# bruAristimunha/Synthetic-Sleep-EEG-Signal-Generation-using-Latent-Diffusion-Models

Measured on AMD Instinct MI355X. Metric: EEG windows/sec (LDM train step), higher is better.
Workload: dtype bf16; 1 GPU; LDM train step on raw (B,1,3072) windows: frozen AutoencoderKL[32,32,64] encode+sample x scale, add_noise, config_ldm.yaml UNet (30.5M params, latent_channels=1) fwd+bwd, epsilon MSE, Adam lr 1e-4 [BASELINE configs[2]/[3]: per-GPU batch 256 = global 2048 / 8]; per_gpu_batch=256, global_batch=256, latent_len=768, parallelism=dp1

## Files before the change

include/eegldm.h:

```cpp
#ifndef EEGLDM_H
#define EEGLDM_H
#include <stdint.h>
#ifdef __cplusplus
extern "C" {
#endif

#define EEGLDM_ABI_VERSION 8

enum { EEGLDM_F32 = 0, EEGLDM_BF16 = 1, EEGLDM_F16 = 2 };
enum {
  EEGLDM_OK = 0,
  EEGLDM_ERR_INVALID = -1,
  EEGLDM_ERR_HIP = -2,
  EEGLDM_ERR_UNSUPPORTED = -3,
  EEGLDM_ERR_NOMEM = -4
};
enum { EEGLDM_PRED_EPSILON = 0, EEGLDM_PRED_V = 1, EEGLDM_PRED_SAMPLE = 2 };

typedef struct eegldm_ctx eegldm_ctx;
typedef struct eegldm_unet eegldm_unet;
typedef struct eegldm_aekl eegldm_aekl;
typedef struct eegldm_disc eegldm_disc;
typedef struct eegldm_block eegldm_block;

int eegldm_abi_version(void);
const char* eegldm_last_error(void);
int eegldm_ctx_create(int hip_device, void* hip_stream, int own_stream, eegldm_ctx** out);
void* eegldm_ctx_stream(const eegldm_ctx*);
int eegldm_ctx_destroy(eegldm_ctx* ctx);
int eegldm_ctx_sync(eegldm_ctx* ctx);
int eegldm_timer_start(eegldm_ctx* ctx);
int eegldm_timer_stop_ms(eegldm_ctx* ctx, float* ms_host);
int eegldm_prof_enable(eegldm_ctx* ctx, int on);
int eegldm_prof_summary(eegldm_ctx* ctx, int kernel_class, double* flops_host, double* ms_host, int* launches_host);
int eegldm_prof_bracket_overhead_ms(eegldm_ctx* ctx, double* ms_host);
int eegldm_prof_dump(eegldm_ctx* ctx, const char* path_host);
int eegldm_debug_reload_env(void);
int eegldm_debug_gn_last_route(int backward, int* out6_host);
int eegldm_debug_bn_last_route(int backward, int* out8_host);
int eegldm_debug_dconv_last_route(int which, int* out8_host);
int eegldm_debug_aekl_last_route(const eegldm_aekl*, int* out10_host);
int eegldm_debug_aekl_encode_route(const eegldm_aekl*, int* out3_host);
int eegldm_debug_pre_conv3(eegldm_ctx*, int dtype, const void* x, const double* in_stats, const float* gamma, const float* beta, const void* w,
                           const float* bias, const void* resid, void* y, double* out_stats, int B, int L, int Cin, int Cout, float eps);
int eegldm_debug_sample_stats(eegldm_ctx*, int dtype, const void* x, long n_per_sample, int B, double* stats);
int eegldm_debug_bn_stats_from_parts(eegldm_ctx*, const float* parts_dev, int nb, float* stats, float* running_mean, float* running_var,
                                     float* num_batches_tracked, long rows, int C);
int eegldm_debug_disc_tail_fwd(eegldm_ctx*, int dtype, const void* y, long ldy, const float* gamma, const float* beta, const float* stats,
                               const float* w3, const float* bias, float slope, float* logits, int B, int L, int C);
int eegldm_debug_disc_tail_bwd(eegldm_ctx*, int dtype, const void* y, long ldy, const float* gamma, const float* beta, const float* stats,
                               const float* w3, float slope, const float* dlogits, void* dy, long lddy, float* dgamma, float* dbeta,
                               float* dw3, float* dbias, int B, int L, int C);
int eegldm_debug_disc_head_bwd(eegldm_ctx*, int dtype, const void* da, long ldda, const void* x, const void* w, const float* bias, float slope,
                               float* dw, float* db, float* dx, int B, int L, int Lo, int C0, int stride);
int eegldm_debug_conv1d_fwd_colstats(eegldm_ctx*, const void* x, long ldx, const void* w, const float* bias, void* y, long ldy,
                                     int B, int Lin, int Cin, int Cout, int K, int stride, int pad_l, int pad_r,
                                     const float* rowvec, long ld_rowvec, const void* resid, long ld_resid, int dtype,
                                     float* col_parts_dev, int* col_nparts_host);

int eegldm_ncl_to_nlc(eegldm_ctx*, const float* src_ncl, void* dst_nlc, long ld_dst, int B, int C, int L, int dst_dtype);
int eegldm_nlc_to_ncl(eegldm_ctx*, const void* src_nlc, long ld_src, float* dst_ncl, int B, int C, int L, int src_dtype);
int eegldm_pack_conv_weight(eegldm_ctx*, const float* w_ref, float* w_packed, int Cout, int Cin, int K);
int eegldm_unpack_conv_weight(eegldm_ctx*, const float* w_packed, float* w_ref, int Cout, int Cin, int K);
int eegldm_cast(eegldm_ctx*, const float* src, void* dst, long n, int dst_dtype);

int eegldm_conv1d_pack_kblocked(eegldm_ctx*, const void* w, void* w_kblocked, int Cout, int Cin, int dtype);
int eegldm_conv1d_pack_kblocked_k(eegldm_ctx*, const void* w, void* w_kblocked, int Cout, int Cin, int K, int dtype);
int eegldm_conv1d_forget_kblocked(eegldm_ctx*, const void* w);
int eegldm_conv1d_pack_stride2(eegldm_ctx*, const void* w, void* w_fwd, void* w_dgrad, int Cout, int Cin, int dtype);
int eegldm_conv1d_pack_dgrad(eegldm_ctx*, const void* w, void* w_dgrad, int Cout, int Cin, int dtype);
int eegldm_conv1d_pack_dgrad_k(eegldm_ctx*, const void* w, void* w_dgrad, int Cout, int Cin, int K, int dtype);
// ... 386 lines not shown
```

synthetic-sleep-eeg-signal-generation-using-latent-diffusion-models_amd/_lib.py:

```python
import ctypes as C
import os

_HERE = os.path.dirname(os.path.abspath(__file__))
LIB_PATH = os.environ.get("EEGLDM_LIB") or os.path.join(_HERE, "libeegldm.so")

F32, BF16, F16 = 0, 1, 2
PRED = {"epsilon": 0, "v_prediction": 1, "sample": 2}


class LibraryMissing(RuntimeError):
    pass


def _load():
    import torch
    if not os.path.exists(LIB_PATH):
        raise LibraryMissing(f"{LIB_PATH} not found: build it with `make` (python -c 'import __graft_entry__ as g; g.build()')")
    return C.CDLL(LIB_PATH)


lib = _load()
lib.eegldm_last_error.restype = C.c_char_p
if hasattr(lib, "eegldm_ctx_stream"):
    lib.eegldm_ctx_stream.restype = C.c_void_p
if hasattr(lib, 'eegldm_unet_num_params'):
    lib.eegldm_unet_num_params.restype = C.c_long

_vp, _i, _l, _f = C.c_void_p, C.c_int, C.c_long, C.c_float
SIGNATURES = {
    "eegldm_abi_version": [],
    "eegldm_last_error": [],
    "eegldm_ctx_create": [_i, _vp, _i, C.POINTER(_vp)],
    "eegldm_ctx_stream": [_vp],
    "eegldm_ctx_destroy": [_vp],
    "eegldm_ctx_sync": [_vp],
    "eegldm_timer_start": [_vp],
    "eegldm_timer_stop_ms": [_vp, C.POINTER(_f)],
    "eegldm_prof_enable": [_vp, _i],
    "eegldm_prof_summary": [_vp, _i, C.POINTER(C.c_double), C.POINTER(C.c_double), C.POINTER(_i)],
    "eegldm_prof_bracket_overhead_ms": [_vp, C.POINTER(C.c_double)],
    "eegldm_prof_dump": [_vp, C.c_char_p],
    "eegldm_debug_reload_env": [],
    "eegldm_debug_gn_last_route": [_i, _vp],
    "eegldm_debug_bn_last_route": [_i, _vp],
    "eegldm_debug_dconv_last_route": [_i, _vp],
    "eegldm_debug_aekl_last_route": [_vp, _vp],
    "eegldm_debug_aekl_encode_route": [_vp, _vp],
    "eegldm_debug_pre_conv3": [_vp, _i, _vp, _vp, _vp, _vp, _vp, _vp, _vp, _vp, _vp, _i, _i, _i, _i, _f],
    "eegldm_debug_sample_stats": [_vp, _i, _vp, _l, _i, _vp],
    "eegldm_debug_bn_stats_from_parts": [_vp, _vp, _i, _vp, _vp, _vp, _vp, _l, _i],
    "eegldm_debug_disc_tail_fwd": [_vp, _i, _vp, _l, _vp, _vp, _vp, _vp, _vp, _f, _vp, _i, _i, _i],
    "eegldm_debug_disc_tail_bwd": [_vp, _i, _vp, _l, _vp, _vp, _vp, _vp, _f, _vp, _vp, _l, _vp, _vp, _vp, _vp, _i, _i, _i],
    "eegldm_debug_disc_head_bwd": [_vp, _i, _vp, _l, _vp, _vp, _vp, _f, _vp, _vp, _vp, _i, _i, _i, _i, _i],
    "eegldm_debug_conv1d_fwd_colstats": [_vp, _vp, _l, _vp, _vp, _vp, _l, _i, _i, _i, _i, _i, _i, _i, _i, _vp, _l, _vp, _l, _i, _vp, _vp],
    "eegldm_ncl_to_nlc": [_vp, _vp, _vp, _l, _i, _i, _i, _i],
    "eegldm_nlc_to_ncl": [_vp, _vp, _l, _vp, _i, _i, _i, _i],
    "eegldm_pack_conv_weight": [_vp, _vp, _vp, _i, _i, _i],
    "eegldm_conv1d_pack_kblocked": [_vp, _vp, _vp, _i, _i, _i],
    "eegldm_conv1d_pack_kblocked_k": [_vp, _vp, _vp, _i, _i, _i, _i],
    "eegldm_batchnorm_lrelu_fwd": [_vp, _vp, _l, _vp, _vp, _vp, _vp, _vp, _vp, _vp, _l, _l, _i, _f, _i, _i],
    "eegldm_batchnorm_lrelu_bwd": [_vp, _vp, _l, _vp, _vp, _vp, _vp, _l, _vp, _l, _vp, _vp, _l, _i, _f, _i],
    "eegldm_kl_reparam_fwd": [_vp, _vp, _vp, _vp, _vp, _vp, _vp, _l, _i, _i],
    "eegldm_kl_reparam_bwd": [_vp, _vp, _vp, _vp, _vp, _vp, _vp, _vp, _l, _f, _i],
    "eegldm_avgpool2_fwd": [_vp, _vp, _l, _vp, _l, _i, _i, _i, _i],
    "eegldm_avgpool2_bwd": [_vp, _vp, _l, _vp, _l, _i, _i, _i, _i],
    "eegldm_nearest2_fwd": [_vp, _vp, _l, _vp, _l, _i, _i, _i, _i],
    "eegldm_nearest2_bwd": [_vp, _vp, _l, _vp, _l, _i, _i, _i, _i],
    "eegldm_conv1d_skip_fwd": [_vp, _vp, _l, _vp, _vp, _vp, _l, _vp, _vp, _vp, _l, _i, _i, _i, _i, _i, _vp, _l, _i],
    "eegldm_comm_unique_id": [_vp],
    "eegldm_comm_create": [_vp, _vp, _i, _i, _vp],
    "eegldm_comm_destroy": [_vp],
    "eegldm_comm_rank": [_vp],
    "eegldm_comm_world": [_vp],
    "eegldm_comm_allreduce_mean_f32": [_vp, _vp, _l, _l],
    "eegldm_comm_broadcast_f32": [_vp, _vp, _l, _i],
    "eegldm_comm_wait": [_vp],
# ... 313 lines not shown
```

synthetic-sleep-eeg-signal-generation-using-latent-diffusion-models_amd/csrc/internal.h:

```cpp
#pragma once
#include "common.h"

int ew_temb(eegldm_ctx*, const int64_t* t, void* out, int B, int dim, int dtype);
int ew_silu(eegldm_ctx*, const float* x, void* y, long n, int dtype);
int ew_silu_bwd(eegldm_ctx*, const float* dy, const float* x, void* dx, long n, int dtype);
int eeg_det_buffer(eegldm_ctx*, size_t bytes, float** out);
int ew_fold_partials_det(eegldm_ctx*, const float* parts, int nparts, long stride, int off, int n, float* total);
int ew_colsum(eegldm_ctx*, const void* x, long ldx, float* out_ps, long ldo, float* total, int B, int L, int C, int dtype);
int ew_softmax(eegldm_ctx*, const float* S, void* P, long rows, int n, int dtype);
int ew_softmax_bwd(eegldm_ctx*, const float* dP, const void* P, void* dS, long rows, int n, float alpha, int dtype);
int ew_add_rows(eegldm_ctx*, void* dst, long ldd, const void* src, long lds, long rows, int C, int dtype);
int ew_dropout_rows(eegldm_ctx*, void* x, long ld, long rows, int C, float p, uint64_t seed, uint64_t offset, int dtype);
int ew_film_silu_fwd(eegldm_ctx*, const void* hn, long ldh, const float* emb, long lde, void* a, long lda, int B, int L, int C, int dtype);
int ew_film_silu_bwd(eegldm_ctx*, const void* hn, long ldh, const float* emb, long lde, const void* da, long ldda, void* dhn, long lddh,
                     float* demb, long ldde, int B, int L, int C, int dtype);
int ew_copy_rows(eegldm_ctx*, void* dst, long ldd, const void* src, long lds, long rows, int C, int dtype);
int ew_ncl2_to_nlc(eegldm_ctx*, const float* x, int Cx, const float* context, int Cc, int rows, void* dst, long ld, int B, int L, int dtype);
int ew_label_emb_add(eegldm_ctx*, float* emb, long ld, const int64_t* y, const float* table, int B, int te, int K);
int ew_label_emb_grad(eegldm_ctx*, const float* demb, long ld, const int64_t* y, int B, int te, int K, float* dtable);
int ew_label_dropout(eegldm_ctx*, const int64_t* y, int64_t* out, int B, float p, int64_t null_class, uint64_t seed, uint64_t offset);
int ew_emb_gather(eegldm_ctx*, const float* table, const int64_t* y, int K, int w, float* out, int B);

bool conv_is_thin(int Cin, int Cout, int dtype);
struct KbDesc { long off; long chunk0; int cout, cin; };
int kblk_pack(eegldm_ctx* ctx, const void* w_plain, void* w_packed, const KbDesc* d_table, int n, long total_chunks);
int kblk_pack_one(eegldm_ctx* ctx, const void* w_plain, void* w_packed, int Cout, int Cin, int taps = 3);
int kblk_pack_t(eegldm_ctx* ctx, const void* w_plain, void* w_packed, const KbDesc* d_table, int n, long total_chunks);
int kblk_pack_t_one(eegldm_ctx* ctx, const void* w_plain, void* w_packed, int Cout, int Cin, int taps = 3);
int s2ws_pack(eegldm_ctx* ctx, const void* w, void* wf, void* wd, int Cout, int Cin);
int dconv_run(eegldm_ctx*, int dtype, bool dgrad, const void* in, long ldin, const void* w, const float* bias,
              const void* resid, long ldr, void* out, long ldout, int B, int Lin, int Lout, int Cin, int Cout, int K,
              int stride, int pad_l, float act_slope = 0.f);
bool dconv_fuses_act(int dtype, int Cin, int Cout, int K, long ldout);
int dconv_wgrad(eegldm_ctx*, int dtype, const void* x, long ldx, const void* dy, long lddy, float* dw, int B, int Lin,
                int Lout, int Cin, int Cout, int K, int stride, int pad_l, float* dbias, int* bias_done);
bool dconv_wgrad_tinyv_ok(int Cin, int Cout, int K);

struct SkinnyGn { const float2* part; const float* gamma; const float* beta; int cpg; float eps; int silu;
                  const float2* part_b = nullptr; int nqa = 0; };
struct SkinnyExt { const void* x2; long ldx2; const void* w2; int Cin2; const float* bias2; };
bool conv_skinny_takes(int dtype, int Cin, int Cout, int taps, int B, int L);
int conv_skinny_ex(eegldm_ctx* ctx, int dtype, const void* x, long ldx, const void* w, int Cin, int Cout, int taps, const float* bias,
                   const float* rowvec, long ld_rowvec, const void* resid, long ldr, void* y, long ldy, int B, int L,
                   const SkinnyGn* gn, float2* part_out, const SkinnyExt* ext = nullptr);
int conv_skinny_try(eegldm_ctx* ctx, int dtype, const void* x, long ldx, const void* w, int Cin, int Cout, int taps, const float* bias,
                    const float* rowvec, long ld_rowvec, const void* resid, long ldr, void* y, long ldy, int B, int L);
int conv_ws2_try(eegldm_ctx*, int dtype, int dgrad, const void* x, const void* w, const float* bias, void* y, int B, int Lo,
                 float* col_parts = nullptr, int* col_nparts = nullptr);
int conv_ws_try(eegldm_ctx*, int dtype, const void* x, long ldx, const void* w, int Cin, int Cout, int transposed, const float* bias,
                const float* rowvec, long ld_rowvec, const void* resid, long ldr, void* y, long ldy, int B, int L,
                float* col_parts = nullptr, int* col_nparts = nullptr);

int op_conv_fwd(eegldm_ctx*, int dtype, const void* x, long ldx, const void* w, const float* bias, void* y, long ldy,
                int B, int Lin, int Cin, int Cout, int K, int stride, int pad_l, int pad_r,
// ... 58 lines not shown
```

synthetic-sleep-eeg-signal-generation-using-latent-diffusion-models_amd/csrc/unet.hip:

```cpp
#include <string.h>

#include <string>
#include <vector>

#include "net.h"

namespace {
constexpr int GN_G = 32;
struct Layer { int kind; ResDesc r; AttnDesc a; RsDesc s; };
inline int layer_cin(const Layer& l) { return l.kind == 0 ? l.r.cin : (l.kind == 1 ? l.a.c : l.s.c); }
inline int layer_cout(const Layer& l) { return l.kind == 0 ? l.r.cout : (l.kind == 1 ? l.a.c : l.s.c); }
inline int layer_len(const Layer& l, int L) {
  if (l.kind == 0) return l.r.updown == 1 ? L / 2 : (l.r.updown == 2 ? L * 2 : L);
  if (l.kind == 2) return l.s.up ? L * 2 : L / 2;
  return L;
}
struct Block { std::vector<Layer> layers; int cin, cout; };
}

struct eegldm_unet : NetBase {
  eegldm_unet_cfg cfg;
  int mc, te;
  long off_emb_w = 0, off_emb_b = 0, off_te0_w, off_te0_b, off_te2_w, off_te2_b, off_cin_w, off_cin_b, off_out_gw, off_out_gb, off_out_w, off_out_b;
  std::vector<Block> in_blocks, out_blocks; Block mid;
// ... 233 lines not shown
extern "C" int eegldm_unet_destroy(eegldm_unet* u) {
  if (!u) return 0;
  sampler_release(u);
  if (u->fuse_stats) (void)hipFree(u->fuse_stats);
  delete u;
  return 0;
}
extern "C" int eegldm_unet_set_dropout(eegldm_unet* u, float p, uint64_t seed) {
  EEG_CHECK(u, "null unet");
  EEG_CHECK(p >= 0.f && p < 1.f, "dropout probability %g outside [0, 1)", (double)p);
  u->dropout = p; u->drop_seed = seed; u->drop_ctr = 0;
  return 0;
}
extern "C" int eegldm_unet_num_entries(const eegldm_unet* u) { return (int)u->entries.size(); }
extern "C" long eegldm_unet_num_params(const eegldm_unet* u) { return u->nparams; }
extern "C" int eegldm_unet_set_grad_hook(eegldm_unet* u, eegldm_grad_hook fn, void* user) {
  EEG_CHECK(u, "null unet");
  u->grad_hook = fn; u->grad_hook_user = user;
  return 0;
}
extern "C" int eegldm_unet_entry(const eegldm_unet* u, int i, char* name, int cap, long* offset, long* numel, int* ndim, int shape[3]) {
  return entry_query(u, i, name, cap, offset, numel, ndim, shape);
}
extern "C" int eegldm_unet_bind(eegldm_unet* u, float* params, float* grads) {
  EEG_CHECK(u && params, "null argument");
  sampler_release(u);
  return u->bind(params, grads);
}
extern "C" int eegldm_unet_sync_weights(eegldm_unet* u) {
  EEG_CHECK(u, "null argument");
  return u->sync_weights();
}

static int embed_chain(eegldm_unet* u, const int64_t* tsteps, const int64_t* labels, int n, float* e0, float* h1e, float* a1e, float* emb,
                       float* semb, float* emb_all) {
  eegldm_ctx* ctx = u->ctx; const int mc = u->mc, te = u->te, F = EEGLDM_F32;
  EEG_TRY(ew_temb(ctx, tsteps, e0, n, mc, F));
  EEG_TRY(op_linear(ctx, F, e0, mc, u->P(u->off_te0_w), mc, u->P(u->off_te0_b), h1e, te, n, te, mc, 1));
  EEG_TRY(ew_silu(ctx, h1e, a1e, (long)n * te, F));
  EEG_TRY(op_linear(ctx, F, a1e, te, u->P(u->off_te2_w), te, u->P(u->off_te2_b), emb, te, n, te, te, 1));
  if (u->num_classes > 0) EEG_TRY(ew_label_emb_add(ctx, emb, te, labels, u->P(u->off_label), n, te, u->num_classes));
  EEG_TRY(ew_silu(ctx, emb, semb, (long)n * te, F));
  return op_linear(ctx, F, semb, te, u->P(u->off_emb_w), te, u->P(u->off_emb_b), emb_all, u->etot, n, u->etot, te, 1);
}
int unet_emb_width(const eegldm_unet* u) { return u->etot; }
long unet_embed_work_floats(const eegldm_unet* u) { return (long)u->mc + 4L * u->te; }
int unet_embed_table(eegldm_unet* u, const int64_t* tsteps_dev, const int64_t* labels_dev, int n, float* table, float* work) {
  EEG_CHECK(u && u->params && tsteps_dev && table && work && n > 0, "bad argument");
  EEG_CHECK(u->num_classes == 0 || labels_dev, "a class-conditional UNet's embedding rows need labels");
  const long te = u->te;
  float* e0 = work; float* h1e = e0 + (long)n * u->mc; float* a1e = h1e + n * te; float* emb = a1e + n * te; float* semb = emb + n * te;
  return embed_chain(u, tsteps_dev, labels_dev, n, e0, h1e, a1e, emb, semb, table);
}
void unet_set_shared_emb(eegldm_unet* u, const float* rows, long ld) { u->emb_shared = rows; u->emb_shared_ld = ld; }

struct LabelArg { const int64_t* y = nullptr; float p_uncond = 0.f; int64_t null_class = 0; uint64_t seed = 0, offset = 0; };
static int unet_forward_impl(eegldm_unet* u, const float* x, const int64_t* tsteps, const LabelArg& lab, float* y, int B, int L, int training) {
  EEG_CHECK(u && x && tsteps && y, "null argument");
  EEG_CHECK(u->params, "bind parameters first");
  EEG_CHECK(B > 0 && L > 0 && (L % (1 << (u->cfg.n_mult - 1))) == 0, "L=%d must be divisible by 2^(levels-1)", L);
  EEG_CHECK(!u->context || B % u->context_rows == 0, "a forward of %d rows cannot share %d context rows (B %% rows != 0)", B, u->context_rows);
  eegldm_ctx* ctx = u->ctx; const int dt = u->dtype; const int mc = u->mc, te = u->te;
  u->arena.reset(); u->rt.clear(); u->at.clear(); u->st.clear(); u->in_out.clear(); u->cat.clear();
  u->B = B; u->L = L; u->have_tape = false; u->training = training != 0;

  {
    EEG_ENV_VAR(bool, no_fuse, getenv("EEGLDM_NO_EVAL_GN_FUSE") != nullptr);
    u->eval_fuse = !training && !no_fuse && (dt == EEGLDM_BF16 || dt == EEGLDM_F16); u->fused_used = false; u->fuse_used = 0; u->part_reg.clear();
    if (u->eval_fuse) {
// ... 63 lines not shown
    EEG_TRY(block_forward(u, u->out_blocks[j], u->cat[j], B, Lj, dst));
    h = dst;
  }
  u->h_last = h;
  ALLOC_OR_FAIL(u->st_out, (float*)u->arena.alloc(sizeof(float) * 2 * B * GN_G));
  ALLOC_OR_FAIL(u->a_out.p, u->alloc_act((long)B * L, mc)); u->a_out.ld = mc; u->a_out.C = mc;
  EEG_TRY(eegldm_groupnorm_fwd(ctx, h.p, h.ld, u->P(u->off_out_gw), u->P(u->off_out_gb), u->a_out.p, mc, u->st_out, B, L, mc, GN_G, GN_EPS, 1, 0, nullptr, 0, dt));
  Arena::Mark mk = u->arena.mark();
  void* yo; ALLOC_OR_FAIL(yo, u->alloc_act((long)B * L, u->cfg.out_channels));
  EEG_TRY(op_conv_fwd(ctx, dt, u->a_out.p, mc, u->W(u->off_out_w), u->P(u->off_out_b), yo, u->cfg.out_channels, B, L, mc, u->cfg.out_channels,
                      3, 1, 1, 1, nullptr, 0, nullptr, 0));
  EEG_TRY(eegldm_nlc_to_ncl(ctx, yo, u->cfg.out_channels, y, B, u->cfg.out_channels, L, dt));
  u->arena.release(mk);
  u->have_tape = !u->fused_used;
  return 0;
}
int unet_forward_labels(eegldm_unet* u, const float* x, const int64_t* t, const int64_t* labels, float* y, int B, int L, int training) {
  LabelArg lab; lab.y = labels;
  return unet_forward_impl(u, x, t, lab, y, B, L, training);
}
extern "C" int eegldm_unet_forward(eegldm_unet* u, const float* x, const int64_t* tsteps, float* y, int B, int L, int training) {
  EEG_CHECK(u, "null unet");
  EEG_CHECK(u->num_classes == 0, "this UNet is class-conditional (%d classes): use eegldm_unet_forward_cond", u->num_classes);
  return unet_forward_impl(u, x, tsteps, LabelArg(), y, B, L, training);
}
extern "C" int eegldm_unet_forward_cond(eegldm_unet* u, const float* x, const int64_t* tsteps, const int64_t* labels, float* y, int B, int L,
                                        int training) {
  EEG_CHECK(u && labels, "null argument");
  EEG_CHECK(u->num_classes > 0, "this UNet was built without classes: use eegldm_unet_forward");
  LabelArg lab; lab.y = labels;
  return unet_forward_impl(u, x, tsteps, lab, y, B, L, training);
}

extern "C" int eegldm_unet_backward(eegldm_unet* u, const float* dy, float* dx_out) {
  EEG_CHECK(u && dy, "null argument");
  EEG_CHECK(u->have_tape, "call eegldm_unet_forward first (with training != 0: an eval-mode forward does not keep the activations)");
  EEG_CHECK(u->grads, "no gradient buffer bound");
  EEG_CHECK(u->num_classes == 0 || u->labels, "the last forward used the sampler's embedding rows: no labels on the tape");
  eegldm_ctx* ctx = u->ctx; const int dt = u->dtype; const int mc = u->mc, te = u->te, B = u->B, L = u->L;
  const int cin = u->cfg.in_channels, cout = u->cfg.out_channels;
  const int n_in = (int)u->in_blocks.size(), n_out = (int)u->out_blocks.size();
  u->have_tape = false;
  u->fold_pending.clear();
  EEG_ENV_VAR(bool, no_grouped, getenv("EEGLDM_NO_GROUPED_WGRAD") != nullptr);
  struct DeferGuard {
    eegldm_ctx* c; bool on;
    DeferGuard(eegldm_ctx* ctx_, bool on_) : c(ctx_), on(on_) { if (on) { c->defer_wgrad = true; c->grp_slot = 0; c->gn_fold_count = 0; c->gn_fold_pending.clear(); } }
    ~DeferGuard() { if (on) { c->defer_wgrad = false; c->wgrad_pending.clear(); c->gn_fold_pending.clear(); } }
  } defer_guard(ctx, !no_grouped && u->param_grads);

  float* demb_all; ALLOC_OR_FAIL(demb_all, (float*)u->arena.alloc(sizeof(float) * (size_t)B * u->etot));
  View dyv; ALLOC_OR_FAIL(dyv.p, u->alloc_act((long)B * L, cout)); dyv.ld = cout;
  EEG_TRY(eegldm_ncl_to_nlc(ctx, dy, dyv.p, cout, B, cout, L, dt));
  EEG_TRY(op_conv_wgrad(ctx, dt, u->a_out.p, mc, dyv.p, cout, u->G(u->off_out_w), u->G(u->off_out_b), B, L, mc, cout, 3, 1, 1, 1));
  View da; ALLOC_OR_FAIL(da.p, u->alloc_act((long)B * L, mc)); da.ld = mc;
  EEG_TRY(op_conv_dgrad(ctx, dt, dyv.p, cout, u->W(u->off_out_w), da.p, mc, B, L, mc, cout, 3, 1, 1, 1, nullptr, 0));
  View dh; ALLOC_OR_FAIL(dh.p, u->alloc_act((long)B * L, mc)); dh.ld = mc; dh.C = mc;
  {
    int gn_deferred = 0;
    EEG_TRY(op_groupnorm_bwd(ctx, u->h_last.p, u->h_last.ld, u->P(u->off_out_gw), u->P(u->off_out_gb), u->st_out, da.p, mc, dh.p, mc,
                             u->G(u->off_out_gw), u->G(u->off_out_gb), B, L, mc, GN_G, 1, 0, nullptr, 0, dt, nullptr, 0, nullptr, nullptr, 0, nullptr,
                             u->param_grads ? &gn_deferred : nullptr));
    if (gn_deferred == 1) EEG_TRY(op_gn_slot_reduce_deferred(ctx, u->G(u->off_out_gw), u->G(u->off_out_gb), mc));
  }
  size_t ri = u->rt.size(), ai = u->at.size();
  std::vector<View> dskip(n_in);
  std::vector<int> in_len(n_in), in_ch(n_in);
  { int Lc = L; in_len[0] = L; in_ch[0] = mc;
    for (int i = 1; i < n_in; i++) { Lc = block_out_len(u->in_blocks[i], Lc); in_len[i] = Lc; in_ch[i] = u->in_blocks[i].cout; } }
  View dout = dh;
  for (int j = n_out - 1; j >= 0; j--) {
    const int i = n_in - 1 - j, C = u->cat[j].C;
    View dcat; ALLOC_OR_FAIL(dcat.p, u->alloc_act((long)B * in_len[i], C)); dcat.ld = C; dcat.C = C;
    EEG_TRY(block_backward(u, u->out_blocks[j], dout, dcat, B, ri, ai, demb_all));
    dout = col_view(dcat, 0, u->skip_c1[j], dt);
    dskip[i] = col_view(dcat, u->skip_c1[j], in_ch[i], dt);
  }
  { View g; ALLOC_OR_FAIL(g.p, u->alloc_act((long)B * in_len[n_in - 1], in_ch[n_in - 1])); g.ld = in_ch[n_in - 1]; g.C = g.ld;
    EEG_TRY(block_backward(u, u->mid, dout, g, B, ri, ai, demb_all, n_in > 1 ? &dskip[n_in - 1] : nullptr, (long)B * in_len[n_in - 1]));
    dout = g; }
  EEG_TRY(u->flush_gn_folds());
  if (u->grad_hook) { EEG_TRY(op_wgrad_flush(ctx)); EEG_TRY(op_gn_fold_flush(ctx)); }
  if (u->grad_hook) EEG_TRY(u->flush_attn_folds());
  if (u->grad_hook) u->grad_hook(u->grad_hook_user, u->off_mid_begin, u->nparams - u->off_mid_begin);
  for (int i = n_in - 1; i >= 1; i--) {
    View g; ALLOC_OR_FAIL(g.p, u->alloc_act((long)B * in_len[i - 1], in_ch[i - 1])); g.ld = in_ch[i - 1]; g.C = g.ld;
    EEG_TRY(block_backward(u, u->in_blocks[i], dout, g, B, ri, ai, demb_all, &dskip[i - 1], (long)B * in_len[i - 1]));
    dout = g;
  }
  if (n_in == 1) EEG_TRY(ew_add_rows(ctx, dout.p, dout.ld, dskip[0].p, dskip[0].ld, (long)B * L, mc, dt));
  EEG_TRY(u->flush_gn_folds());
  EEG_TRY(op_conv_wgrad(ctx, dt, u->x0.p, u->x0.ld, dout.p, dout.ld, u->G(u->off_cin_w), u->G(u->off_cin_b), B, L, cin, mc, 3, 1, 1, 1));
  if (dx_out) {
    void* dx0; ALLOC_OR_FAIL(dx0, u->alloc_act((long)B * L, cin));
    EEG_TRY(op_conv_dgrad(ctx, dt, dout.p, dout.ld, u->W(u->off_cin_w), dx0, cin, B, L, cin, mc, 3, 1, 1, 1, nullptr, 0));
    EEG_TRY(eegldm_nlc_to_ncl(ctx, dx0, cin, dx_out, B, cin - u->context_channels, L, dt));
  }
  const int E = u->etot, F = EEGLDM_F32;
  auto fbuf = [&](long n) { return (float*)u->arena.alloc(sizeof(float) * (size_t)n); };
  EEG_TRY(ew_colsum(ctx, demb_all, E, nullptr, 0, u->G(u->off_emb_b), 1, B, E, F));
  EEG_TRY(op_linear_wgrad(ctx, F, u->semb, te, demb_all, E, u->G(u->off_emb_w), te, B, E, te));
  float* dsemb; ALLOC_OR_FAIL(dsemb, fbuf((long)B * te));
  EEG_TRY(op_linear_dgrad(ctx, F, demb_all, E, u->P(u->off_emb_w), te, dsemb, te, B, E, te, 1));
  float* demb; ALLOC_OR_FAIL(demb, fbuf((long)B * te));
  EEG_TRY(ew_silu_bwd(ctx, dsemb, u->emb, demb, (long)B * te, F));
  if (u->num_classes > 0) EEG_TRY(ew_label_emb_grad(ctx, demb, te, u->labels, B, te, u->num_classes, u->G(u->off_label)));
  EEG_TRY(ew_colsum(ctx, demb, te, nullptr, 0, u->G(u->off_te2_b), 1, B, te, F));
  EEG_TRY(op_linear_wgrad(ctx, F, u->a1e, te, demb, te, u->G(u->off_te2_w), te, B, te, te));
  float* da1; ALLOC_OR_FAIL(da1, fbuf((long)B * te));
  EEG_TRY(op_linear_dgrad(ctx, F, demb, te, u->P(u->off_te2_w), te, da1, te, B, te, te, 1));
  float* dh1; ALLOC_OR_FAIL(dh1, fbuf((long)B * te));
  EEG_TRY(ew_silu_bwd(ctx, da1, u->h1e, dh1, (long)B * te, F));
  EEG_TRY(ew_colsum(ctx, dh1, te, nullptr, 0, u->G(u->off_te0_b), 1, B, te, F));
  EEG_TRY(op_linear_wgrad(ctx, F, u->e0, mc, dh1, te, u->G(u->off_te0_w), mc, B, te, mc));
  EEG_TRY(op_wgrad_flush(ctx));
  EEG_TRY(u->flush_attn_folds());
  EEG_TRY(op_gn_fold_flush(ctx));
  return 0;
}

struct CtxArg { const float *src, *mask; float p_none, p_prefix; int span_min, span_max; uint64_t seed, offset; float* mask_out; };
static int ldm_train_step(eegldm_unet* u, const float* latents, const float* noise, const int64_t* t, const float* acp,
                          int pred_type, int B, int L, float grad_scale, float* loss, const LabelArg& lab, bool weighted = false,
                          const float* wtab = nullptr, float* per_sample = nullptr, const CtxArg* cx = nullptr) {
  EEG_CHECK(u && latents && noise && t && acp && loss, "null argument");
  EEG_CHECK(pred_type == EEGLDM_PRED_EPSILON || pred_type == EEGLDM_PRED_V, "prediction type must be epsilon or v_prediction");
  eegldm_ctx* ctx = u->ctx;
  const int C = u->cfg.in_channels - u->context_channels;
  EEG_CHECK(cx || u->context_channels == 0, "this UNet takes a context (%d channels): use eegldm_ldm_train_step_ctx", u->context_channels);
  EEG_CHECK(u->cfg.out_channels == C, "LDM training needs x channels == out_channels");
  const long n = (long)B * C * L, nctx = cx ? (long)B * (C + 1) * L : 0;
  static thread_local float* stage = nullptr; static thread_local size_t stage_cap = 0;
  if (stage_cap < (size_t)(n * 4 + nctx)) {
    if (stage) hipFree(stage);
    stage = nullptr; stage_cap = 0;
    HIP_TRY(hipMalloc(&stage, sizeof(float) * (n * 4 + nctx))); stage_cap = (size_t)(n * 4 + nctx);
  }
  float *noisy = stage, *pred = stage + n, *target = stage + 2 * n, *dpred = stage + 3 * n, *context = stage + 4 * n;
  struct ClearContext { eegldm_unet* u; ~ClearContext() { if (u) { u->context = nullptr; u->context_rows = 0; } } } clear_context{cx ? u : nullptr};
  if (cx) {
    EEG_TRY(eegldm_add_noise_context(ctx, latents, cx->src, noise, t, acp, cx->mask, cx->p_none, cx->p_prefix, cx->span_min, cx->span_max, cx->seed,
                                     cx->offset, noisy, context, cx->mask_out, B, C, L));
    u->context = context; u->context_rows = B;
  } else EEG_TRY(eegldm_add_noise(ctx, latents, noise, t, acp, noisy, B, (long)C * L));
  EEG_TRY(unet_forward_impl(u, noisy, t, lab, pred, B, L, 1));
  if (weighted) {
    EEG_TRY(eegldm_diffusion_loss(ctx, pred, latents, noise, t, acp, wtab, pred_type, B, (long)C * L, grad_scale, loss, per_sample, dpred));
    return eegldm_unet_backward(u, dpred, nullptr);
  }
  const float* tgt = noise;
  if (pred_type == EEGLDM_PRED_V) { EEG_TRY(eegldm_get_velocity(ctx, latents, noise, t, acp, target, B, (long)C * L)); tgt = target; }
// ... 51 lines not shown
```

Baseline: 15760 windows/s.

## Fuse timestep-embedding MLP forward/backward into custom MFMA GEMM kernels with epilogues

```diff
diff --git a/include/eegldm.h b/include/eegldm.h
--- a/include/eegldm.h
+++ b/include/eegldm.h
@@ -37,6 +37,11 @@
 int eegldm_prof_dump(eegldm_ctx* ctx, const char* path_host);
 int eegldm_debug_reload_env(void);
 int eegldm_debug_gn_last_route(int backward, int* out6_host);
+int eegldm_debug_emb_mlp_launches(long* out_host, int reset);
+int eegldm_debug_emb_mlp_plan(int n, int mc, int te, int E, int* out12_host);
+int eegldm_debug_unet_embed(eegldm_unet* u, const int64_t* tsteps_dev, const int64_t* labels_dev, int n, float* table, float* work);
+int eegldm_debug_unet_embed_backward(eegldm_unet* u, const int64_t* labels_dev, int n, const float* demb_all, const float* work,
+                                     float* dsemb_out);
 int eegldm_debug_bn_last_route(int backward, int* out8_host);
 int eegldm_debug_dconv_last_route(int which, int* out8_host);
 int eegldm_debug_aekl_last_route(const eegldm_aekl*, int* out10_host);
diff --git a/synthetic-sleep-eeg-signal-generation-using-latent-diffusion-models_amd/_lib.py b/synthetic-sleep-eeg-signal-generation-using-latent-diffusion-models_amd/_lib.py
--- a/synthetic-sleep-eeg-signal-generation-using-latent-diffusion-models_amd/_lib.py
+++ b/synthetic-sleep-eeg-signal-generation-using-latent-diffusion-models_amd/_lib.py
@@ -42,6 +42,10 @@
     "eegldm_prof_dump": [_vp, C.c_char_p],
     "eegldm_debug_reload_env": [],
     "eegldm_debug_gn_last_route": [_i, _vp],
+    "eegldm_debug_emb_mlp_launches": [_vp, _i],
+    "eegldm_debug_emb_mlp_plan": [_i, _i, _i, _i, _vp],
+    "eegldm_debug_unet_embed": [_vp, _vp, _vp, _i, _vp, _vp],
+    "eegldm_debug_unet_embed_backward": [_vp, _vp, _i, _vp, _vp, _vp],
     "eegldm_debug_bn_last_route": [_i, _vp],
     "eegldm_debug_dconv_last_route": [_i, _vp],
     "eegldm_debug_aekl_last_route": [_vp, _vp],
diff --git a/synthetic-sleep-eeg-signal-generation-using-latent-diffusion-models_amd/csrc/emb_mlp.hip b/synthetic-sleep-eeg-signal-generation-using-latent-diffusion-models_amd/csrc/emb_mlp.hip
--- /dev/null
+++ b/synthetic-sleep-eeg-signal-generation-using-latent-diffusion-models_amd/csrc/emb_mlp.hip
@@ -0,0 +1,317 @@
+#include "emb_mlp_plan.h"
+#include "internal.h"
+
+namespace {
+
+enum { EPI_FWD = 0, EPI_PART = 1, EPI_DSILU = 2, EPI_WGRAD = 3 };
+
+struct EmbGemm {
+  const float* A; long lda; const float* B; long ldb;
+  int M, N, K;
+  int avec, bvec;
+  int tiles_n;
+  float* C; long ldc;
+  float* C2;
+  const float* bias;
+  const int64_t* labels; const float* table; int num_classes;
+  const float* aux; long ldaux;
+  float* colsum;
+  const float* zero;
+  int kper; long part_stride;
+};
+
+__device__ __forceinline__ float4 ld4(const float* __restrict__ base, long off, bool ok, bool vec, const float* __restrict__ zero) {
+  const float* p = ok ? base + off : zero;
+  if (vec) return *(const float4*)p;
+  return make_float4(p[0], p[1], p[2], p[3]);
+}
+template <bool KM, int T> struct TileMap {
+  static constexpr int PITCH = KM ? T + 4 : EMB_KC + 4;
+  static constexpr int W4 = KM ? T / 4 : EMB_KC / 4, NV = T / 16, STEP = 256 / W4;
+  static __device__ __forceinline__ int o(int tid, int i) { return tid / W4 + STEP * i; }
+  static __device__ __forceinline__ int q(int tid) { return (tid % W4) * 4; }
+};
+template <bool KM, int T>
+__device__ __forceinline__ void load_tile(float4 (&r)[T / 16], const float* __restrict__ X, long ld, bool vec, int x0, int xend, int k0, int kend, int tid,
+                                          const float* __restrict__ zero) {
+  using M = TileMap<KM, T>;
+  const int q = M::q(tid);
+#pragma unroll
+  for (int i = 0; i < M::NV; i++) {
+    const int o = M::o(tid, i);
+    if constexpr (KM) { const int k = k0 + o, x = x0 + q; r[i] = ld4(X, (long)k * ld + x, k < kend && emb_valid4(x, xend) == 4, vec, zero); }
+    else { const int x = x0 + o, k = k0 + q; r[i] = ld4(X, (long)x * ld + k, x < xend && emb_valid4(k, kend) == 4, vec, zero); }
+  }
+}
+template <bool KM, int T> __device__ __forceinline__ void store_tile(float* __restrict__ s, const float4 (&r)[T / 16], int tid) {
+  using M = TileMap<KM, T>;
+#pragma unroll
+  for (int i = 0; i < M::NV; i++) *(float4*)(s + M::o(tid, i) * M::PITCH + M::q(tid)) = r[i];
+}
+template <bool KM, int T> __device__ __forceinline__ float4 frag(const float* __restrict__ s, int x, int g, int h) {
+  constexpr int P = TileMap<KM, T>::PITCH;
+  if constexpr (KM) {
+    const float* p = s + (16 * g + 4 * h) * P + x;
+    return make_float4(p[0], p[P], p[2 * P], p[3 * P]);
+  } else return *(const float4*)(s + x * P + 16 * g + 4 * h);
+}
+
+template <bool A_KM, bool B_KM, int EPI, int T>
+__global__ __launch_bounds__(256) void emb_gemm_kernel(const EmbGemm p0, const EmbGemm p1, int tiles0) {
+  constexpr int FR = T / 32, NV = T / 16;
+  __shared__ __attribute__((aligned(16))) float As[EMB_KC * (T + 4)];
+  __shared__ __attribute__((aligned(16))) float Bs[EMB_KC * (T + 4)];
+  int bid = blockIdx.x;
+  { const int nb = gridDim.x; if ((nb & 7) == 0) bid = (bid & 7) * (nb >> 3) + (bid >> 3); }
+  const bool second = EPI == EPI_WGRAD && bid >= tiles0;
+  const EmbGemm& p = second ? p1 : p0;
+  if (second) bid -= tiles0;
+  const int tiles_m = (p.M + T - 1) / T, per_split = tiles_m * p.tiles_n;
+  const int z = bid / per_split;
+  bid -= z * per_split;
+  int tm, tn;
+  if constexpr (EPI == EPI_WGRAD) { tm = bid / p.tiles_n; tn = bid - tm * p.tiles_n; }
+  else { tn = bid / tiles_m; tm = bid - tn * tiles_m; }
+  const int m0 = tm * T, n0 = tn * T;
+  int kbeg = 0, kend = p.K;
+  if constexpr (EPI == EPI_PART) { kbeg = z * p.kper; kend = min(p.K, kbeg + p.kper); }
+  const int tid = threadIdx.x, lane = tid & 63, w = tid >> 6, c = lane & 15, h = lane >> 4, wm = w & 1, wn = w >> 1;
+
+  f32x4 acc[FR][FR];
+#pragma unroll
+  for (int i = 0; i < FR; i++)
+#pragma unroll
+    for (int j = 0; j < FR; j++) acc[i][j] = f32x4{0.f, 0.f, 0.f, 0.f};
+  float4 ra[2][NV], rb[2][NV];
+  float cs = 0.f;
+  const bool do_colsum = EPI == EPI_WGRAD && tn == 0 && p.colsum != nullptr;
+  const bool avec = p.avec != 0, bvec = p.bvec != 0;
+
+  auto stage = [&](float4 (&qa)[NV], float4 (&qb)[NV], int k0) {
+    __syncthreads();
+    store_tile<A_KM, T>(As, qa, tid);
+    store_tile<B_KM, T>(Bs, qb, tid);
+    __syncthreads();
+    if (k0 + 2 * EMB_KC < kend) {
+      load_tile<A_KM, T>(qa, p.A, p.lda, avec, m0, p.M, k0 + 2 * EMB_KC, kend, tid, p.zero);
+      load_tile<B_KM, T>(qb, p.B, p.ldb, bvec, n0, p.N, k0 + 2 * EMB_KC, kend, tid, p.zero);
+    }
+    if constexpr (EPI == EPI_WGRAD) {
+      if (do_colsum && tid < T) {
+#pragma unroll 8
+        for (int k = 0; k < EMB_KC; k++) cs += As[k * (T + 4) + tid];
+      }
+    }
+#pragma unroll
+    for (int g = 0; g < EMB_KC / 16; g++) {
+      float4 a[FR], b[FR];
+#pragma unroll
+      for (int i = 0; i < FR; i++) a[i] = frag<A_KM, T>(As, wm * (T / 2) + i * 16 + c, g, h);
+#pragma unroll
+      for (int j = 0; j < FR; j++) b[j] = frag<B_KM, T>(Bs, wn * (T / 2) + j * 16 + c, g, h);
+#pragma unroll
+      for (int i = 0; i < FR; i++)
+#pragma unroll
+        for (int j = 0; j < FR; j++) {
+          acc[i][j] = __builtin_amdgcn_mfma_f32_16x16x4f32(a[i].x, b[j].x, acc[i][j], 0, 0, 0);
+          acc[i][j] = __builtin_amdgcn_mfma_f32_16x16x4f32(a[i].y, b[j].y, acc[i][j], 0, 0, 0);
+          acc[i][j] = __builtin_amdgcn_mfma_f32_16x16x4f32(a[i].z, b[j].z, acc[i][j], 0, 0, 0);
+          acc[i][j] = __builtin_amdgcn_mfma_f32_16x16x4f32(a[i].w, b[j].w, acc[i][j], 0, 0, 0);
+        }
+    }
+  };
+
+  load_tile<A_KM, T>(ra[0], p.A, p.lda, avec, m0, p.M, kbeg, kend, tid, p.zero);
+  load_tile<B_KM, T>(rb[0], p.B, p.ldb, bvec, n0, p.N, kbeg, kend, tid, p.zero);
+  if (kbeg + EMB_KC < kend) {
+    load_tile<A_KM, T>(ra[1], p.A, p.lda, avec, m0, p.M, kbeg + EMB_KC, kend, tid, p.zero);
+    load_tile<B_KM, T>(rb[1], p.B, p.ldb, bvec, n0, p.N, kbeg + EMB_KC, kend, tid, p.zero);
+  }
+  for (int k0 = kbeg; k0 < kend; k0 += 2 * EMB_KC) {
+    stage(ra[0], rb[0], k0);
+    if (k0 + EMB_KC < kend) stage(ra[1], rb[1], k0 + EMB_KC);
+  }
+
+  int nn[FR]; bool nok[FR]; float bias[FR];
+#pragma unroll
+  for (int j = 0; j < FR; j++) {
+    const int n = n0 + wn * (T / 2) + j * 16 + c;
+    nok[j] = n < p.N; nn[j] = nok[j] ? n : p.N - 1; bias[j] = 0.f;
+    if constexpr (EPI == EPI_FWD) bias[j] = p.bias[nn[j]];
+  }
+  long at[FR][4][FR]; bool ok[FR][4][FR]; float ex[FR][4][FR]; bool lok[FR][4];
+#pragma unroll
+  for (int i = 0; i < FR; i++)
+#pragma unroll
+    for (int r = 0; r < 4; r++) {
+      const int m = m0 + wm * (T / 2) + i * 16 + 4 * h + r;
+      const bool mok = m < p.M; const int mm = mok ? m : p.M - 1;
+      long lab = -1; lok[i][r] = false;
+      if constexpr (EPI == EPI_FWD) {
+        if (p.labels) { lab = (long)p.labels[mm]; lok[i][r] = lab >= 0 && lab < p.num_classes; if (!lok[i][r]) lab = 0; }
+      }
+#pragma unroll
+      for (int j = 0; j < FR; j++) {
+        ok[i][r][j] = mok && nok[j]; at[i][r][j] = (long)mm * p.ldc + nn[j]; ex[i][r][j] = 0.f;
+        if constexpr (EPI == EPI_FWD) { if (p.labels) ex[i][r][j] = p.table[lab * p.N + nn[j]]; }
+        else if constexpr (EPI == EPI_DSILU) ex[i][r][j] = p.aux[(long)mm * p.ldaux + nn[j]];
+        else if constexpr (EPI == EPI_WGRAD) ex[i][r][j] = p.C[at[i][r][j]];
+      }
+    }
+#pragma unroll
+  for (int i = 0; i < FR; i++)
+#pragma unroll
+    for (int r = 0; r < 4; r++)
+#pragma unroll
+      for (int j = 0; j < FR; j++) {
+        if (!ok[i][r][j]) continue;
+        const float v = acc[i][j][r];
+        const long o_at = at[i][r][j];
+        if constexpr (EPI == EPI_FWD) {
+          float o = v + bias[j];
+          if (lok[i][r]) o += ex[i][r][j];
+          p.C[o_at] = o;
+          if (p.C2) p.C2[o_at] = silu_f(o);
+        } else if constexpr (EPI == EPI_PART) p.C[(long)z * p.part_stride + o_at] = v;
+        else if constexpr (EPI == EPI_DSILU) p.C[o_at] = v * silu_grad_f(ex[i][r][j]);
+        else p.C[o_at] = ex[i][r][j] + v;
+      }
+  if constexpr (EPI == EPI_WGRAD) {
+    if (do_colsum && tid < T && m0 + tid < p.M) p.colsum[m0 + tid] += cs;
+  }
+}
+
+__global__ __launch_bounds__(256) void emb_fold_silu_kernel(const float* __restrict__ part, int nparts, long stride, const float* __restrict__ x,
+                                                            float* __restrict__ dsemb, float* __restrict__ demb, long n) {
+  const long i = (long)blockIdx.x * 256 + threadIdx.x;
+  if (i >= n) return;
+  float s = part[i];
+#pragma unroll 4
+  for (int z = 1; z < nparts; z++) s += part[(long)z * stride + i];
+  if (dsemb) dsemb[i] = s;
+  demb[i] = s * silu_grad_f(x[i]);
+}
+
+std::atomic<long> g_launches{0};
+
+inline int vec_ok(const float* p, long ld) { return ((uintptr_t)p & 15) == 0 && (ld & 3) == 0; }
+int pick_tile(long tiles64) {
+  EEG_ENV_VAR(int, forced, getenv("EEGLDM_EMB_MLP_TILE") ? atoi(getenv("EEGLDM_EMB_MLP_TILE")) : 0);
+  return forced == 32 || forced == 64 ? forced : emb_pick_tile(tiles64);
+}
+EmbGemm problem(const float* A, long lda, const float* B, long ldb, int M, int N, int K, float* C, long ldc) {
+  EmbGemm g = {};
+  g.A = A; g.lda = lda; g.B = B; g.ldb = ldb; g.M = M; g.N = N; g.K = K; g.C = C; g.ldc = ldc;
+  g.avec = vec_ok(A, lda); g.bvec = vec_ok(B, ldb); g.kper = K;
+  return g;
+}
+inline int tiles_of(const EmbGemm& g, int T) { return emb_tiles(g.M, T) * emb_tiles(g.N, T); }
+
+template <bool A_KM, bool B_KM, int EPI>
+int launch(eegldm_ctx* ctx, const EmbGemm& p0, const EmbGemm* p1, int splits) {
+  const int T = EPI == EPI_PART ? EMB_TILE : pick_tile((long)tiles_of(p0, EMB_TILE) + (p1 ? tiles_of(*p1, EMB_TILE) : 0));
+  const int t0 = tiles_of(p0, T), total = t0 + (p1 ? tiles_of(*p1, T) : 0);
+  EmbGemm a = p0, b = p1 ? *p1 : p0;
+  a.tiles_n = emb_tiles(a.N, T); b.tiles_n = emb_tiles(b.N, T);
+  a.zero = b.zero = (const float*)ctx->zero_page;
+  if (T == 32) hipLaunchKernelGGL((emb_gemm_kernel<A_KM, B_KM, EPI, 32>), dim3(total * splits), dim3(256), 0, ctx->stream, a, b, t0);
+  else hipLaunchKernelGGL((emb_gemm_kernel<A_KM, B_KM, EPI, 64>), dim3(total * splits), dim3(256), 0, ctx->stream, a, b, t0);
+  g_launches.fetch_add(1, std::memory_order_relaxed);
+  LAUNCH_CHECK();
+  return 0;
+}
+
+}
+
+bool emb_mlp_enabled() {
+  EEG_ENV_VAR(bool, off, getenv("EEGLDM_NO_EMB_MLP") != nullptr);
+  return !off;
+}
+bool emb_mlp_takes(const EmbMlpNet& net, int n) {
+  return n > 0 && net.mc > 0 && net.te > 0 && net.E > 0 && (net.mc & 3) == 0 && (net.te & 3) == 0 && (net.E & 3) == 0;
+}
+
+int emb_mlp_fwd(eegldm_ctx* ctx, const EmbMlpNet& net, const int64_t* tsteps, const int64_t* labels, int n, const EmbMlpTape& tp, float* emb_all) {
+  const int mc = net.mc, te = net.te, E = net.E;
+  EEG_CHECK(emb_mlp_takes(net, n), "shape not served (n %d, mc %d, te %d, E %d)", n, mc, te, E);
+  EEG_TRY(ew_temb(ctx, tsteps, tp.e0, n, mc, EEGLDM_F32));
+  {
+    EmbGemm g = problem(tp.e0, mc, net.w0, mc, n, te, mc, tp.h1e, te);
+    g.bias = net.b0; g.C2 = tp.a1e;
+    EEG_TRY((launch<false, false, EPI_FWD>(ctx, g, nullptr, 1)));
+  }
+  {
+    EmbGemm g = problem(tp.a1e, te, net.w2, te, n, te, te, tp.emb, te);
+    g.bias = net.b2; g.C2 = tp.semb;
+    if (net.num_classes > 0) { g.labels = labels; g.table = net.label; g.num_classes = net.num_classes; }
+    EEG_TRY((launch<false, false, EPI_FWD>(ctx, g, nullptr, 1)));
+  }
+  {
+    EmbGemm g = problem(tp.semb, te, net.we, te, n, E, te, emb_all, E);
+    g.bias = net.be;
+    EEG_TRY((launch<false, false, EPI_FWD>(ctx, g, nullptr, 1)));
+  }
+  return 0;
+}
+
+long emb_mlp_bwd_work_floats(const EmbMlpNet& net, int n) {
+  int splits, kper;
+  emb_splitk_plan(emb_tiles(n) * emb_tiles(net.te), net.E, &splits, &kper);
+  return ((long)splits + 2) * n * net.te;
+}
+int emb_mlp_bwd(eegldm_ctx* ctx, const EmbMlpNet& net, const EmbMlpGrads& gr, const int64_t* labels, int n, const EmbMlpTape& tp,
+                const float* demb_all, float* work, float* dsemb_out) {
+  const int mc = net.mc, te = net.te, E = net.E;
+  EEG_CHECK(emb_mlp_takes(net, n), "shape not served (n %d, mc %d, te %d, E %d)", n, mc, te, E);
+  int splits, kper;
+  emb_splitk_plan(emb_tiles(n) * emb_tiles(te), E, &splits, &kper);
+  const long nte = (long)n * te;
+  float* part = work; float* demb = work + (long)splits * nte; float* dh1 = demb + nte;
+  {
+    EmbGemm g = problem(demb_all, E, tp.semb, te, E, te, n, gr.we, te);
+    g.colsum = gr.be;
+    EEG_TRY((launch<true, true, EPI_WGRAD>(ctx, g, nullptr, 1)));
+  }
+  {
+    EmbGemm g = problem(demb_all, E, net.we, te, n, te, E, part, te);
+    g.kper = kper; g.part_stride = nte;
+    EEG_TRY((launch<false, true, EPI_PART>(ctx, g, nullptr, splits)));
+  }
+  hipLaunchKernelGGL(emb_fold_silu_kernel, dim3((unsigned)((nte + 255) / 256)), dim3(256), 0, ctx->stream, part, splits, nte, tp.emb, dsemb_out, demb, nte);
+  g_launches.fetch_add(1, std::memory_order_relaxed);
+  LAUNCH_CHECK();
+  if (net.num_classes > 0) EEG_TRY(ew_label_emb_grad(ctx, demb, te, labels, n, te, net.num_classes, gr.label));
+  {
+    EmbGemm g = problem(demb, te, net.w2, te, n, te, te, dh1, te);
+    g.aux = tp.h1e; g.ldaux = te;
+    EEG_TRY((launch<false, true, EPI_DSILU>(ctx, g, nullptr, 1)));
+  }
+  {
+    EmbGemm g2 = problem(demb, te, tp.a1e, te, te, te, n, gr.w2, te);
+    g2.colsum = gr.b2;
+    EmbGemm g0 = problem(dh1, te, tp.e0, mc, te, mc, n, gr.w0, mc);
+    g0.colsum = gr.b0;
+    EEG_TRY((launch<true, true, EPI_WGRAD>(ctx, g2, &g0, 1)));
+  }
+  return 0;
+}
+
+extern "C" int eegldm_debug_emb_mlp_launches(long* out_host, int reset) {
+  EEG_CHECK(out_host, "null argument");
+  *out_host = reset ? g_launches.exchange(0) : g_launches.load();
+  return 0;
+}
+extern "C" int eegldm_debug_emb_mlp_plan(int n, int mc, int te, int E, int* out12_host) {
+  EEG_CHECK(out12_host && n > 0 && mc > 0 && te > 0 && E > 0, "bad argument");
+  int splits, kper;
+  emb_splitk_plan(emb_tiles(n) * emb_tiles(te), E, &splits, &kper);
+  EmbMlpNet net = {}; net.mc = mc; net.te = te; net.E = E;
+  const long wf = emb_mlp_bwd_work_floats(net, n);
+  auto tiles = [](int M, int N, int T) { return emb_tiles(M, T) * emb_tiles(N, T); };
+  auto picked = [&](int M, int N) { return tiles(M, N, emb_pick_tile(tiles(M, N, EMB_TILE))); };
+  const int tp = emb_pick_tile((long)tiles(te, te, EMB_TILE) + tiles(te, mc, EMB_TILE));
+  const int v[12] = {picked(n, te), picked(n, te), picked(n, E), picked(E, te), tiles(te, te, tp), tiles(te, mc, tp), tiles(n, te, EMB_TILE), splits, kper,
+                     picked(n, te), (int)(wf & 0x7fffffff), (int)(wf >> 31)};
+  for (int i = 0; i < 12; i++) out12_host[i] = v[i];
+  return 0;
+}
diff --git a/synthetic-sleep-eeg-signal-generation-using-latent-diffusion-models_amd/csrc/emb_mlp_plan.h b/synthetic-sleep-eeg-signal-generation-using-latent-diffusion-models_amd/csrc/emb_mlp_plan.h
--- /dev/null
+++ b/synthetic-sleep-eeg-signal-generation-using-latent-diffusion-models_amd/csrc/emb_mlp_plan.h
@@ -0,0 +1,27 @@
+#pragma once
+#ifdef __HIPCC__
+#define EMB_HD __host__ __device__
+#else
+#define EMB_HD
+#endif
+
+constexpr int EMB_TILE = 64;
+constexpr int EMB_KC = 64;
+constexpr int EMB_MAX_SPLIT = 32;
+constexpr int EMB_SPLIT_TARGET = 512;
+
+static inline int emb_tiles(int n, int tile = EMB_TILE) { return (n + tile - 1) / tile; }
+constexpr int EMB_SMALL_GRID = 128;
+static inline int emb_pick_tile(long tiles64) { return tiles64 < EMB_SMALL_GRID ? 32 : 64; }
+
+static inline void emb_splitk_plan(int tiles, int K, int* splits, int* kper) {
+  const int chunks = (K + EMB_KC - 1) / EMB_KC;
+  int want = tiles > 0 ? (EMB_SPLIT_TARGET + tiles - 1) / tiles : 1;
+  if (want > EMB_MAX_SPLIT) want = EMB_MAX_SPLIT;
+  if (want > chunks) want = chunks;
+  if (want < 1) want = 1;
+  const int per = (chunks + want - 1) / want;
+  *kper = per * EMB_KC;
+  *splits = (chunks + per - 1) / per;
+}
+EMB_HD static inline int emb_valid4(int i, int end) { const int v = end - i; return v < 0 ? 0 : (v > 4 ? 4 : v); }
diff --git a/synthetic-sleep-eeg-signal-generation-using-latent-diffusion-models_amd/csrc/internal.h b/synthetic-sleep-eeg-signal-generation-using-latent-diffusion-models_amd/csrc/internal.h
--- a/synthetic-sleep-eeg-signal-generation-using-latent-diffusion-models_amd/csrc/internal.h
+++ b/synthetic-sleep-eeg-signal-generation-using-latent-diffusion-models_amd/csrc/internal.h
@@ -20,6 +20,16 @@
 int ew_label_emb_grad(eegldm_ctx*, const float* demb, long ld, const int64_t* y, int B, int te, int K, float* dtable);
 int ew_label_dropout(eegldm_ctx*, const int64_t* y, int64_t* out, int B, float p, int64_t null_class, uint64_t seed, uint64_t offset);
 int ew_emb_gather(eegldm_ctx*, const float* table, const int64_t* y, int K, int w, float* out, int B);
+
+struct EmbMlpNet { const float *w0, *b0, *w2, *b2, *we, *be, *label; int mc, te, E, num_classes; };
+struct EmbMlpGrads { float *w0, *b0, *w2, *b2, *we, *be, *label; };
+struct EmbMlpTape { float *e0, *h1e, *a1e, *emb, *semb; };
+bool emb_mlp_enabled();
+bool emb_mlp_takes(const EmbMlpNet&, int n);
+int emb_mlp_fwd(eegldm_ctx*, const EmbMlpNet&, const int64_t* tsteps, const int64_t* labels, int n, const EmbMlpTape&, float* emb_all);
+long emb_mlp_bwd_work_floats(const EmbMlpNet&, int n);
+int emb_mlp_bwd(eegldm_ctx*, const EmbMlpNet&, const EmbMlpGrads&, const int64_t* labels, int n, const EmbMlpTape&, const float* demb_all,
+                float* work, float* dsemb_out);
 
 bool conv_is_thin(int Cin, int Cout, int dtype);
 struct KbDesc { long off; long chunk0; int cout, cin; };
diff --git a/synthetic-sleep-eeg-signal-generation-using-latent-diffusion-models_amd/csrc/unet.hip b/synthetic-sleep-eeg-signal-generation-using-latent-diffusion-models_amd/csrc/unet.hip
--- a/synthetic-sleep-eeg-signal-generation-using-latent-diffusion-models_amd/csrc/unet.hip
+++ b/synthetic-sleep-eeg-signal-generation-using-latent-diffusion-models_amd/csrc/unet.hip
@@ -289,9 +289,20 @@
   return u->sync_weights();
 }
 
+static EmbMlpNet emb_net(const eegldm_unet* u) {
+  EmbMlpNet net = {};
+  net.w0 = u->P(u->off_te0_w); net.b0 = u->P(u->off_te0_b); net.w2 = u->P(u->off_te2_w); net.b2 = u->P(u->off_te2_b);
+  net.we = u->P(u->off_emb_w); net.be = u->P(u->off_emb_b); net.label = u->num_classes > 0 ? u->P(u->off_label) : nullptr;
+  net.mc = u->mc; net.te = u->te; net.E = u->etot; net.num_classes = u->num_classes;
+  return net;
+}
 static int embed_chain(eegldm_unet* u, const int64_t* tsteps, const int64_t* labels, int n, float* e0, float* h1e, float* a1e, float* emb,
                        float* semb, float* emb_all) {
   eegldm_ctx* ctx = u->ctx; const int mc = u->mc, te = u->te, F = EEGLDM_F32;
+  {
+    const EmbMlpNet net = emb_net(u);
+    if (emb_mlp_enabled() && emb_mlp_takes(net, n)) return emb_mlp_fwd(ctx, net, tsteps, labels, n, EmbMlpTape{e0, h1e, a1e, emb, semb}, emb_all);
+  }
   EEG_TRY(ew_temb(ctx, tsteps, e0, n, mc, F));
   EEG_TRY(op_linear(ctx, F, e0, mc, u->P(u->off_te0_w), mc, u->P(u->off_te0_b), h1e, te, n, te, mc, 1));
   EEG_TRY(ew_silu(ctx, h1e, a1e, (long)n * te, F));
@@ -421,6 +432,38 @@
   return unet_forward_impl(u, x, tsteps, lab, y, B, L, training);
 }
 
+static int embed_chain_backward(eegldm_unet* u, const int64_t* labels, int B, const EmbMlpTape& tp, const float* demb_all, float* dsemb_out) {
+  eegldm_ctx* ctx = u->ctx; const int mc = u->mc, te = u->te;
+  {
+    const EmbMlpNet net = emb_net(u);
+    if (emb_mlp_enabled() && emb_mlp_takes(net, B)) {
+      float* work; ALLOC_OR_FAIL(work, (float*)u->arena.alloc(sizeof(float) * (size_t)emb_mlp_bwd_work_floats(net, B)));
+      const EmbMlpGrads gr = {u->G(u->off_te0_w), u->G(u->off_te0_b), u->G(u->off_te2_w), u->G(u->off_te2_b), u->G(u->off_emb_w), u->G(u->off_emb_b),
+                              u->num_classes > 0 ? u->G(u->off_label) : nullptr};
+      return emb_mlp_bwd(ctx, net, gr, labels, B, tp, demb_all, work, dsemb_out);
+    }
+  }
+  const int E = u->etot, F = EEGLDM_F32;
+  auto fbuf = [&](long n) { return (float*)u->arena.alloc(sizeof(float) * (size_t)n); };
+  EEG_TRY(ew_colsum(ctx, demb_all, E, nullptr, 0, u->G(u->off_emb_b), 1, B, E, F));
+  EEG_TRY(op_linear_wgrad(ctx, F, tp.semb, te, demb_all, E, u->G(u->off_emb_w), te, B, E, te));
+  float* dsemb; ALLOC_OR_FAIL(dsemb, fbuf((long)B * te));
+  EEG_TRY(op_linear_dgrad(ctx, F, demb_all, E, u->P(u->off_emb_w), te, dsemb, te, B, E, te, 1));
+  float* demb; ALLOC_OR_FAIL(demb, fbuf((long)B * te));
+  if (dsemb_out) HIP_TRY(hipMemcpyAsync(dsemb_out, dsemb, sizeof(float) * (size_t)B * te, hipMemcpyDeviceToDevice, ctx->stream));
+  EEG_TRY(ew_silu_bwd(ctx, dsemb, tp.emb, demb, (long)B * te, F));
+  if (u->num_classes > 0) EEG_TRY(ew_label_emb_grad(ctx, demb, te, labels, B, te, u->num_classes, u->G(u->off_label)));
+  EEG_TRY(ew_colsum(ctx, demb, te, nullptr, 0, u->G(u->off_te2_b), 1, B, te, F));
+  EEG_TRY(op_linear_wgrad(ctx, F, tp.a1e, te, demb, te, u->G(u->off_te2_w), te, B, te, te));
+  float* da1; ALLOC_OR_FAIL(da1, fbuf((long)B * te));
+  EEG_TRY(op_linear_dgrad(ctx, F, demb, te, u->P(u->off_te2_w), te, da1, te, B, te, te, 1));
+  float* dh1; ALLOC_OR_FAIL(dh1, fbuf((long)B * te));
+  EEG_TRY(ew_silu_bwd(ctx, da1, tp.h1e, dh1, (long)B * te, F));
+  EEG_TRY(ew_colsum(ctx, dh1, te, nullptr, 0, u->G(u->off_te0_b), 1, B, te, F));
+  EEG_TRY(op_linear_wgrad(ctx, F, tp.e0, mc, dh1, te, u->G(u->off_te0_w), mc, B, te, mc));
+  return 0;
+}
+
 extern "C" int eegldm_unet_backward(eegldm_unet* u, const float* dy, float* dx_out) {
   EEG_CHECK(u && dy, "null argument");
   EEG_CHECK(u->have_tape, "call eegldm_unet_forward first (with training != 0: an eval-mode forward does not keep the activations)");
@@ -485,27 +528,24 @@
     EEG_TRY(op_conv_dgrad(ctx, dt, dout.p, dout.ld, u->W(u->off_cin_w), dx0, cin, B, L, cin, mc, 3, 1, 1, 1, nullptr, 0));
     EEG_TRY(eegldm_nlc_to_ncl(ctx, dx0, cin, dx_out, B, cin - u->context_channels, L, dt));
   }
-  const int E = u->etot, F = EEGLDM_F32;
-  auto fbuf = [&](long n) { return (float*)u->arena.alloc(sizeof(float) * (size_t)n); };
-  EEG_TRY(ew_colsum(ctx, demb_all, E, nullptr, 0, u->G(u->off_emb_b), 1, B, E, F));
-  EEG_TRY(op_linear_wgrad(ctx, F, u->semb, te, demb_all, E, u->G(u->off_emb_w), te, B, E, te));
-  float* dsemb; ALLOC_OR_FAIL(dsemb, fbuf((long)B * te));
-  EEG_TRY(op_linear_dgrad(ctx, F, demb_all, E, u->P(u->off_emb_w), te, dsemb, te, B, E, te, 1));
-  float* demb; ALLOC_OR_FAIL(demb, fbuf((long)B * te));
-  EEG_TRY(ew_silu_bwd(ctx, dsemb, u->emb, demb, (long)B * te, F));
-  if (u->num_classes > 0) EEG_TRY(ew_label_emb_grad(ctx, demb, te, u->labels, B, te, u->num_classes, u->G(u->off_label)));
-  EEG_TRY(ew_colsum(ctx, demb, te, nullptr, 0, u->G(u->off_te2_b), 1, B, te, F));
-  EEG_TRY(op_linear_wgrad(ctx, F, u->a1e, te, demb, te, u->G(u->off_te2_w), te, B, te, te));
-  float* da1; ALLOC_OR_FAIL(da1, fbuf((long)B * te));
-  EEG_TRY(op_linear_dgrad(ctx, F, demb, te, u->P(u->off_te2_w), te, da1, te, B, te, te, 1));
-  float* dh1; ALLOC_OR_FAIL(dh1, fbuf((long)B * te));
-  EEG_TRY(ew_silu_bwd(ctx, da1, u->h1e, dh1, (long)B * te, F));
-  EEG_TRY(ew_colsum(ctx, dh1, te, nullptr, 0, u->G(u->off_te0_b), 1, B, te, F));
-  EEG_TRY(op_linear_wgrad(ctx, F, u->e0, mc, dh1, te, u->G(u->off_te0_w), mc, B, te, mc));
+  EEG_TRY(embed_chain_backward(u, u->labels, B, EmbMlpTape{u->e0, u->h1e, u->a1e, u->emb, u->semb}, demb_all, nullptr));
   EEG_TRY(op_wgrad_flush(ctx));
   EEG_TRY(u->flush_attn_folds());
   EEG_TRY(op_gn_fold_flush(ctx));
   return 0;
+}
+
+extern "C" int eegldm_debug_unet_embed(eegldm_unet* u, const int64_t* tsteps_dev, const int64_t* labels_dev, int n, float* table, float* work) {
+  return unet_embed_table(u, tsteps_dev, labels_dev, n, table, work);
+}
+extern "C" int eegldm_debug_unet_embed_backward(eegldm_unet* u, const int64_t* labels_dev, int n, const float* demb_all, const float* work,
+                                                float* dsemb_out) {
+  EEG_CHECK(u && u->params && u->grads && demb_all && work && n > 0, "bad argument (parameters and gradients must be bound)");
+  EEG_CHECK(u->num_classes == 0 || labels_dev, "a class-conditional UNet's embedding backward needs labels");
+  const long te = u->te;
+  float* e0 = const_cast<float*>(work); float* h1e = e0 + (long)n * u->mc; float* a1e = h1e + n * te; float* emb = a1e + n * te; float* semb = emb + n * te;
+  u->arena.reset(); u->have_tape = false;
+  return embed_chain_backward(u, labels_dev, n, EmbMlpTape{e0, h1e, a1e, emb, semb}, demb_all, dsemb_out);
 }
 
 struct CtxArg { const float *src, *mask; float p_none, p_prefix; int span_min, span_max; uint64_t seed, offset; float* mask_out; };
```

Result: faster. 15940 windows/s, median of 6 (+1.1%).
